# jhamrick/gaussian_processes

Hardware: AMD Instinct MI355X
Metric: GP fit+predict wall-clock (kernel build + Cholesky + solve + log_lh + posterior mean) (lower is better)
Workload: dtype f64; 1 GPU; N=65536 d=32 RBF(GaussianKernel) f64, m=1000 test points, h=1 w=0.5*sqrt(d) s=1; N=65536, d=32, m=1000, parallelism=1 GPU

## Files before the change

### gaussian_processes_amd/_lib.py

```python
import ctypes
import os
from ctypes import (POINTER, c_char_p, c_double, c_float, c_int, c_int64, c_size_t,
                    c_uint64, c_void_p)

import numpy as np

_HERE = os.path.dirname(os.path.abspath(__file__))
LIB_PATH = os.path.join(_HERE, "libgpx.so")

OK = 0
ERR_ARG, ERR_HIP, ERR_NO_DEVICE, ERR_NOMEM, ERR_UNSUPPORTED, ERR_INTERNAL = -1, -2, -3, -4, -5, -6
(ROUTE_TRSV_OPS, ROUTE_TRSV_STEPS, ROUTE_PANEL_RES, ROUTE_PANEL_CHAIN, ROUTE_FIT_RIDE, ROUTE_FIT_TWO_SOLVES,
 ROUTE_GEMM_FAST, ROUTE_GEMM_GENERIC, ROUTE_SYRK_EXACT, ROUTE_SYRK_PATCH, ROUTE_MG_BCAST_ONE, ROUTE_MG_BCAST_SAG,
 ROUTE_FIT_OPS_AHEAD, ROUTE_TRSM_OPS, ROUTE_POTRF_PAIR, ROUTE_VAR_CHUNK, ROUTE_LOO_CHUNK, ROUTE_TRSM_L_OPS,
 ROUTE_GRAD_CHUNK) = range(19)
F64, F32 = 0, 1
KERNEL_GAUSSIAN, KERNEL_PERIODIC, KERNEL_GAUSSIAN_ARD = 0, 1, 2
ARD_MAX_D = 64
FULL, LOWER = 0, 1
(K, DK_DH, DK_DW, DK_DP, D2K_DHDH, D2K_DHDW, D2K_DHDP, D2K_DWDW, D2K_DWDP, D2K_DPDP) = range(10)
MIN_LOG = -705.6238298100243

MEMBER_BY_NAME = {
    "K": K, "dK_dh": DK_DH, "dK_dw": DK_DW, "dK_dp": DK_DP,
    "d2K_dhdh": D2K_DHDH, "d2K_dhdw": D2K_DHDW, "d2K_dwdh": D2K_DHDW,
    "d2K_dhdp": D2K_DHDP, "d2K_dpdh": D2K_DHDP, "d2K_dwdw": D2K_DWDW,
    "d2K_dwdp": D2K_DWDP, "d2K_dpdw": D2K_DWDP, "d2K_dpdp": D2K_DPDP,
}

MG_ID_BYTES = 128
MG_BCAST_FN = ctypes.CFUNCTYPE(c_int, c_void_p, c_void_p, c_size_t, c_int, c_void_p)
MG_ALLREDUCE_FN = ctypes.CFUNCTYPE(c_int, c_void_p, c_void_p, c_size_t, c_int, c_int, c_void_p)

c_double_p = POINTER(c_double)
c_int_p = POINTER(c_int)

_SIGNATURES = {
    "gpx_version": (c_int, []),
    "gpx_last_error": (c_char_p, []),
    "gpx_device_count": (c_int, [c_int_p]),
    "gpx_set_device": (c_int, [c_int]),
    "gpx_get_device": (c_int, [c_int_p]),
    "gpx_device_info": (c_int, [c_int, c_char_p, c_size_t, c_int_p, c_int_p, POINTER(c_uint64)]),
    "gpx_malloc": (c_int, [POINTER(c_void_p), c_size_t]),
    "gpx_free": (c_int, [c_void_p]),
    "gpx_mem_info": (c_int, [ctypes.POINTER(c_size_t), ctypes.POINTER(c_size_t)]),
    "gpx_memcpy_h2d": (c_int, [c_void_p, c_void_p, c_size_t, c_void_p]),
    "gpx_memcpy_d2h": (c_int, [c_void_p, c_void_p, c_size_t, c_void_p]),
# ... 249 lines not shown
```

### gaussian_processes_amd/csrc/gpx_common.h

```cpp
#pragma once
#include <hip/hip_runtime.h>
#include <stdint.h>
#include <stdio.h>
#include <stdlib.h>
#include <string.h>
#include <math.h>
#include <vector>

#include "../../include/gpx.h"
#include "gpx_tune.h"

namespace gpx {

void set_error(const char *fmt, ...);
int  hip_fail(hipError_t e, const char *what, const char *file, int line);
int  ensure_device();

#define GPX_HIP(call)                                                        \
    do {                                                                     \
        hipError_t e__ = (call);                                             \
        if (e__ != hipSuccess) return gpx::hip_fail(e__, #call, __FILE__, __LINE__); \
    } while (0)

#define GPX_TRY(call)                                                        \
    do {                                                                     \
        int rc__ = (call);                                                   \
        if (rc__ != GPX_OK) return rc__;                                     \
    } while (0)

#define GPX_ARG(cond, msg)                                                   \
    do {                                                                     \
        if (!(cond)) { gpx::set_error("%s: %s", __func__, msg); return GPX_ERR_ARG; } \
    } while (0)

#define GPX_LAUNCH_CHECK()                                                   \
    do {                                                                     \
        hipError_t e__ = hipGetLastError();                                  \
        if (e__ != hipSuccess) return gpx::hip_fail(e__, "kernel launch", __FILE__, __LINE__); \
    } while (0)


enum Route { RT_TRSV_OPS = 0, RT_TRSV_STEPS = 1, RT_PANEL_RES = 2, RT_PANEL_CHAIN = 3, RT_FIT_RIDE = 4,
             RT_FIT_TWO_SOLVES = 5, RT_GEMM_FAST = 6, RT_GEMM_GENERIC = 7, RT_SYRK_EXACT = 8, RT_SYRK_PATCH = 9,
             RT_MG_BCAST_ONE = 10, RT_MG_BCAST_SAG = 11, RT_FIT_OPS_AHEAD = 12, RT_TRSM_OPS = 13, RT_POTRF_PAIR = 14, RT_VAR_CHUNK = 15, RT_LOO_CHUNK = 16,
             RT_TRSM_L_OPS = 17, RT_GRAD_CHUNK = 18, RT_COUNT = 19 };
void route_hit(int route);

int check_internal_info(int info);

static inline hipStream_t S(void *s) { return (hipStream_t)s; }
static inline size_t esize(int dtype) { return dtype == GPX_F64 ? 8 : 4; }
static inline int64_t round_up(int64_t v, int64_t m) { return (v + m - 1) / m * m; }
static inline int64_t cdiv(int64_t a, int64_t b) { return (a + b - 1) / b; }

static inline int order(hipEvent_t e, hipStream_t from, hipStream_t to)
{
    GPX_HIP(hipEventRecord(e, from));
    GPX_HIP(hipStreamWaitEvent(to, e, 0));
    return GPX_OK;
}
struct EventPool {
    std::vector<hipEvent_t> ev; size_t next = 0;
    int reserve(size_t count)
    {
        while (ev.size() < count) {
            hipEvent_t x;
            GPX_HIP(hipEventCreateWithFlags(&x, hipEventDisableTiming));
            ev.push_back(x);
        }
        return GPX_OK;
    }
    int get(hipEvent_t *e) { GPX_TRY(reserve(next + 1)); *e = ev[next++]; return GPX_OK; }
    void rewind() { next = 0; }
    void destroy() { for (hipEvent_t e : ev) (void)hipEventDestroy(e); ev.clear(); next = 0; }
    int order(hipStream_t from, hipStream_t to) { hipEvent_t e; GPX_TRY(get(&e)); return gpx::order(e, from, to); }
};

enum ProfClass { PC_KMAT = 0, PC_GEMM = 1, PC_POTRF_DIAG = 2, PC_TRSM_ROWS = 3, PC_TRSV = 4,
// ... 60 lines not shown
int syrk_bc(int dtype, int64_t n, int64_t row_begin, void *Cloc, int64_t ldc, int64_t cl0, int64_t cl1,
            const void *Pb, int64_t ldp, int64_t k0, int64_t kb, int64_t nb, int P, int rank,
            hipStream_t st, const int *abort_flag = nullptr, const Batch *bt = nullptr);
struct PanelHints { bool idle_chip = false; int leaf_force = 0; };
struct PotrfHook { int (*fn)(void *user, int64_t cols_done, hipEvent_t panel_done); void *user; };
int potrf_panel(int dtype, void *A, int64_t lda, int64_t n, int64_t r0, int64_t c0, int64_t kb,
                int *info_dev, hipStream_t st, const Batch *bt = nullptr, int64_t kpre = 0,
                hipEvent_t done = nullptr, PanelHints hints = {});
int potrf(int dtype, void *A, int64_t n, int64_t lda, int *info_dev, hipStream_t st, const Batch *bt = nullptr,
          int64_t xrows = 0,
          bool may_block = false,
          const PotrfHook *hook = nullptr);
int potrf_panel_res(int dtype, void *A, int64_t lda, int64_t n, int64_t r0, int64_t c0, int64_t kb, int *info_dev,
                    hipStream_t st, const Batch *bt = nullptr, int64_t kpre = 0, hipEvent_t done = nullptr, PanelHints hints = {});
int64_t panel_res_max();
hipStream_t potrf_side_stream();
bool kernel_values_finite(int kernel, const double *p, double s, int dtype);
bool panel_res_fold(int64_t rows, int64_t kpre, int64_t kb, size_t es, int64_t lda, const void *base);
constexpr int TRSV_OPS_BLOCK = 512;
static inline int64_t trsv_ops_nblocks(int64_t n) { return n / TRSV_OPS_BLOCK; }
static inline bool trsv_ops_whole_blocks(int64_t n) { return n >= TRSV_OPS_BLOCK && n % TRSV_OPS_BLOCK == 0; }
struct TrsvOps {
    GrowBuf mem;
    bool valid = false;
    int64_t built = 0;
    void invalidate() { valid = false; built = 0; }
    static TrsvOps view(void *p, size_t bytes) { TrsvOps o; o.mem.p = p; o.mem.bytes = bytes; return o; }
};
int trsv_ops_build(int dtype, const void *L, int64_t n, int64_t ldl, TrsvOps *ops, hipStream_t st);
bool trsv_ops_ahead_ok(int dtype, const void *L, int64_t n, int64_t ldl);
bool trsm_ops_ok(int dtype, const void *L, int64_t n, int64_t ldl);
size_t trsv_ops_bytes(int dtype, int64_t n);
int trsv_ops_build_upto(int dtype, const void *L, int64_t n, int64_t ldl, TrsvOps *ops, int64_t kend, hipStream_t st);
int trsv_lower(int dtype, const void *L, int64_t n, int64_t ldl, void *b, void *x, int transpose,
               hipStream_t st, const Batch *bt = nullptr,
               TrsvOps *ops = nullptr);
int trsm_right_lt(int dtype, const void *L, int64_t n, int64_t ldl, void *X, int64_t m, int64_t ldx,
                  hipStream_t st, int x_upper = 0, TrsvOps *ops = nullptr,
                  int64_t c0 = 0);
int trsm_right_l(int dtype, const void *L, int64_t n, int64_t ldl, void *X, int64_t m, int64_t ldx, hipStream_t st,
                 TrsvOps *ops = nullptr);
int pred_grad(int dtype, int kernel, const void *xo, int64_t m, const void *x, int64_t n, int d, const double *params,
              const void *alpha, const void *B, int64_t ldb, double scale, const double *col_div, double *out_dev, hipStream_t st);
int inv_from_factor(int dtype, const void *L, int64_t n, int64_t ldl, void *X, void *W, int tri, hipStream_t st,
                    TrsvOps *ops, int count = 1, int64_t sL = 0, void *group_ops = nullptr);
int logdet_chol(int dtype, const void *L, int64_t n, int64_t ldl, double *out_dev, hipStream_t st, int count = 1,
                int64_t sL = 0, int64_t so = 0);
int dot(int dtype, const void *a, const void *b, int64_t n, double *out_dev, hipStream_t st, int count = 1,
        int64_t sa = 0, int64_t sb = 0, int64_t so = 0);
int tril(int dtype, void *A, int64_t n, int64_t lda, hipStream_t st);
int var_rows(int dtype, int kernel, const void *X, int64_t rows, int64_t n, int64_t ldx, const void *xo, int d,
             const double *params, const double *kdiag_dev, int accumulate, double *out_dev, hipStream_t st);
int var_finish(int dtype, int kernel, const void *xo, int d, const double *params, const double *acc_dev, int64_t rows,
               double *out_dev, hipStream_t st);
int eye_rows(int dtype, void *X, int64_t rows, int64_t ld, int64_t c0, int64_t cz, hipStream_t st);
int loo_rows(int dtype, const void *X, int64_t rows, int64_t n, int64_t ldx, int64_t c0, const void *y, const void *alpha,
             double *kii, double *mean, double *var, double *logp, hipStream_t st);
int loo_points(int dtype, const double *kii, const void *y, const void *alpha, int64_t n, double *mean, double *var, double *logp,
               hipStream_t st);
int sum_f64(const double *a, int64_t n, double *out_dev, hipStream_t st);
int var_plan(int dtype, int64_t n, int64_t m, int64_t chunk_rows, size_t free_bytes, int64_t *rows, int64_t *chunks, size_t *bytes);
int dloglh_reduce(int dtype, int kernel, const void *x, int64_t n, int d, const double *params,
                  const void *alpha, const void *W, int64_t ldw, double *partial_dev, double *out4,
                  hipStream_t st);
int scale_points(int dtype, const void *x, int64_t n, int d, const double *w_host, void *out, hipStream_t st);
void ard_iso(const double *params, int d, double *iso2);
// ... 8 lines not shown
```

### gaussian_processes_amd/csrc/gpx_gp.hip

```cpp
#include "gpx_common.h"
#include <cmath>
#include <vector>

#include "gpx_gp_internal.h"

namespace gpx {

template <typename T>
__global__ void cvt_from_f64(const double *__restrict__ src, T *__restrict__ dst, int64_t n)
{
    const int64_t i = (int64_t)blockIdx.x * blockDim.x + threadIdx.x;
    if (i < n) dst[i] = (T)src[i];
}

template <typename T>
__global__ void cvt_to_f64_2d(const T *__restrict__ src, int64_t lds, double *__restrict__ dst,
                              int64_t ldd, int64_t rows, int64_t cols, int lower_only)
{
    const int64_t c = (int64_t)blockIdx.x * blockDim.x + threadIdx.x;
    if (c >= cols) return;
    for (int64_t r = blockIdx.y; r < rows; r += gridDim.y) {
        const double v = (double)src[r * lds + c];
        dst[r * ldd + c] = (lower_only && c > r) ? 0.0 : v;
    }
// ... 250 lines not shown
int gpx_gp_get_params(gpx_gp_t *g, double *params, int cap, int *count)
{
    GP_ENTER(g);
    GPX_ARG(g->have_params, "no kernel parameters in the handle");
    GPX_ARG(cap >= 0 && (cap == 0 || params), "bad arguments");
    if (count) *count = g->nparams;
    for (int i = 0; i < g->nparams && i < cap; ++i) params[i] = g->params[i];
    return GPX_OK;
}

int gpx_gp_set_K(gpx_gp_t *g, const double *Kxx, int64_t ld)
{
    GP_ENTER(g);
    GPX_ARG(g && Kxx && ld >= g->n, "bad arguments");
    const int64_t n = g->n;
    if (g->dtype == GPX_F64) {
        GPX_HIP(hipMemcpy2DAsync(g->A, (size_t)g->lda * 8, Kxx, (size_t)ld * 8, (size_t)n * 8, (size_t)n,
                                 hipMemcpyHostToDevice, g->st));
        GPX_HIP(hipStreamSynchronize(g->st));
    } else {
        DevBuf tmp;
        GPX_TRY(tmp.alloc((size_t)n * n * 8));
        GPX_HIP(hipMemcpy2DAsync(tmp.p, (size_t)n * 8, Kxx, (size_t)ld * 8, (size_t)n * 8, (size_t)n,
                                 hipMemcpyHostToDevice, g->st));
        for (int64_t r = 0; r < n; ++r)
            hipLaunchKernelGGL((cvt_from_f64<float>), dim3((unsigned)cdiv(n, 256)), dim3(256), 0, g->st,
                               (const double *)tmp.p + r * n, (float *)g->A + r * g->lda, n);
        GPX_HIP(hipStreamSynchronize(g->st));
    }
    g->have_K = true; g->fitted = false; g->have_kii = false;
    return GPX_OK;
}

struct OpsAhead { gpx_gp *g; int64_t group, last; };
static int ops_ahead_step(void *user, int64_t cols_done, hipEvent_t panel_done)
{
    OpsAhead *o = (OpsAhead *)user;
    gpx_gp *g = o->g;
    const int64_t ready = std::min(trsv_ops_nblocks(cols_done), o->last);
    if (ready - g->ops.built < o->group) return GPX_OK;
    GPX_HIP(hipStreamWaitEvent(g->st_ops, panel_done, 0));
    return trsv_ops_build_upto(g->dtype, g->A, g->n, g->lda, &g->ops, ready, g->st_ops);
}

int gpx_gp_fit(gpx_gp_t *g, int *info)
{
    GP_ENTER(g);
    GPX_ARG(g, "gp is NULL");
    GPX_ARG(g->have_data && (g->have_params || g->have_K),
            "set_data and set_params (or set_K) must be called before fit");
    const GpView v = gp_view(g);
    if (!g->have_K && (!g->x_finite || !kernel_values_finite(v.kernel, v.params, g->s, g->dtype))) {
        set_error("%s (%s)", NONFINITE_MSG, g->x_finite ? "kernel parameters or s" : "x");
        return GPX_ERR_ARG;
    }
    const size_t es = esize(g->dtype);
    int *info_dev = (int *)(g->scal + 3);
    hipStream_t st = g->st;
    GPX_HIP(hipEventRecord(g->ev[0], st));
    if (!g->have_K)
        GPX_TRY(kmat(g->dtype, v.kernel, GPX_K, v.x, g->n, v.x, g->n, g->d, v.params, g->s * g->s,
                     GPX_LOWER, g->A, g->lda, st));
    g->have_K = false;
    g->have_kii = false;
    GPX_HIP(hipEventRecord(g->ev[1], st));
    const int64_t ride_max = tune().fit_ride_max;
    const bool ride = g->n <= ride_max;
    route_hit(ride ? RT_FIT_RIDE : RT_FIT_TWO_SOLVES);
    char *row_n = (char *)g->A + (size_t)g->n * g->lda * es;
    if (ride) GPX_HIP(hipMemcpyAsync(row_n, g->y, (size_t)g->n * es, hipMemcpyDeviceToDevice, st));
    g->ops.invalidate();
    const bool ahead = tune().fit_ops_ahead != 0 && g->n >= tune().fit_ops_ahead_min &&
                       trsv_ops_ahead_ok(g->dtype, g->A, g->n, g->lda);
    const int64_t nfull = trsv_ops_nblocks(g->n), tail = tune().fit_ops_tail;
    const int64_t group = std::max<int64_t>(1, std::min(nfull, nfull - tail));
    OpsAhead oa = {g, group, std::max<int64_t>(0, nfull - tail)};
    PotrfHook hook = {ops_ahead_step, &oa};
    if (ahead) {
        if (!g->st_ops) {
            int least = 0, greatest = 0;
            GPX_HIP(hipDeviceGetStreamPriorityRange(&least, &greatest));
            GPX_HIP(hipStreamCreateWithPriority(&g->st_ops, hipStreamNonBlocking, least));
            GPX_HIP(hipEventCreateWithFlags(&g->ev_ops, hipEventDisableTiming));
        }
        GPX_TRY(g->ops.mem.reserve(trsv_ops_bytes(g->dtype, g->n), st));
        GPX_TRY(order(g->ev_ops, st, g->st_ops));
    }
    GPX_TRY(potrf(g->dtype, g->A, g->n, g->lda, info_dev, st, nullptr, ride ? 1 : 0, true, ahead ? &hook : nullptr));
    if (ahead) {
        GPX_TRY(order(g->ev_ops, g->st_ops, st));
        if (g->ops.built > 0) route_hit(RT_FIT_OPS_AHEAD);
    }
    GPX_HIP(hipEventRecord(g->ev[2], st));
    if (ride) {
        GPX_TRY(trsv_lower(g->dtype, g->A, g->n, g->lda, row_n, g->alpha, 1, st, nullptr, &g->ops));
    } else {
        GPX_HIP(hipMemcpyAsync(g->t0, g->y, (size_t)g->n * es, hipMemcpyDeviceToDevice, st));
        GPX_TRY(trsv_lower(g->dtype, g->A, g->n, g->lda, g->t0, g->t1, 0, st, nullptr, &g->ops));
        GPX_TRY(trsv_lower(g->dtype, g->A, g->n, g->lda, g->t1, g->alpha, 1, st, nullptr, &g->ops));
    }
    GPX_HIP(hipEventRecord(g->ev[3], st));
    GPX_TRY(logdet_chol(g->dtype, g->A, g->n, g->lda, g->scal + 0, st));
    GPX_TRY(dot(g->dtype, g->y, g->alpha, g->n, g->scal + 1, st));
    GPX_HIP(hipEventRecord(g->ev[4], st));
    g->fitted = true;
    if (info) {
        GPX_HIP(hipMemcpyAsync(info, info_dev, sizeof(int), hipMemcpyDeviceToHost, st));
        GPX_HIP(hipStreamSynchronize(st));
        GPX_TRY(check_internal_info(*info));
    }
    return GPX_OK;
}

static int gp_scalars(gpx_gp_t *g, double *logdet, double *yta, int *info)
{
    GP_ENTER(g);
    GPX_ARG(g && g->fitted, "gp is not fitted");
    double h[4];
    GPX_HIP(hipMemcpyAsync(h, g->scal, sizeof(h), hipMemcpyDeviceToHost, g->st));
    GPX_HIP(hipStreamSynchronize(g->st));
    int inf;
    memcpy(&inf, &h[3], sizeof(int));
    GPX_TRY(check_internal_info(inf));
    if (logdet) *logdet = h[0];
    if (yta) *yta = h[1];
    if (info) *info = inf;
    return GPX_OK;
}
// ... 743 lines not shown
```

### gaussian_processes_amd/csrc/gpx_gp_internal.h

```cpp
#pragma once
#include "gpx_common.h"

struct gpx_gp {
    int device;
    int dtype, kernel, d, nparams;
    int64_t n, lda;
    void *x, *y, *A, *alpha, *t0, *t1;
    void *xs;
    double *scal;
    hipStream_t st;
    hipEvent_t ev[6];
    double params[1 + GPX_ARD_MAX_D];
    double iso[2];
    double s;
    bool have_data, have_params, fitted, have_K;
    bool x_finite, y_finite;
    float ms[5];
    gpx::GrowBuf bw; int64_t bw_cap;
    gpx::TrsvOps ops;
    gpx::GrowBuf gw; int64_t gw_cap;
    gpx::TrsvOps bops;
    double *kii;
    bool have_kii;
    hipStream_t st_ops;
    hipEvent_t ev_ops;
};

namespace gpx {
int gp_scan_finite(gpx_gp *g);
static inline int nparams_of(int kernel, int d) { return kernel == GPX_KERNEL_GAUSSIAN_ARD ? 1 + d : (kernel == GPX_KERNEL_PERIODIC ? 3 : 2); }
struct GpView { int kernel; const void *x; const double *params; };
static inline GpView gp_view(const gpx_gp *g)
{
    if (g->kernel == GPX_KERNEL_GAUSSIAN_ARD) return {GPX_KERNEL_GAUSSIAN, g->xs, g->iso};
    return {g->kernel, g->x, g->params};
}
int gp_rescale(gpx_gp *g);
}

#define GP_ENTER(g)                                                          \
    GPX_ARG((g) != nullptr, "gp is NULL");                                   \
    gpx::tune_refresh();                                                     \
    gpx::DeviceGuard guard__((g)->device);                                   \
    if (guard__.rc != GPX_OK) return guard__.rc;                             \
    gpx::StreamTurn turn__((g)->st);                                         \
    gpx::RoctxRange api_range__(__func__)
```

### gaussian_processes_amd/csrc/gpx_mg.hip

```cpp
#include "gpx_common.h"
#include <dlfcn.h>
#include <climits>
#include <cmath>
#include <vector>

extern "C" {
typedef struct ncclComm *ncclComm_t;
typedef struct { char internal[128]; } ncclUniqueId;
typedef int ncclResult_t;
typedef int ncclDataType_t;
typedef int ncclRedOp_t;
}
static constexpr ncclResult_t ncclSuccess = 0;
static constexpr ncclDataType_t ncclInt32 = 2, ncclFloat32 = 7, ncclFloat64 = 8;
static constexpr ncclRedOp_t ncclSum = 0, ncclMax = 2;
static_assert(sizeof(ncclUniqueId) == GPX_MG_ID_BYTES, "ncclUniqueId is 128 bytes");

extern "C" int gpx_d_mean(int dtype, int kernel, const void *xo, int64_t m, const void *x, int64_t n, int d,
                          const double *params, const void *alpha, void *out, void *stream);
namespace gpx {

struct Rccl {
    void *lib = nullptr;
    ncclResult_t (*GetUniqueId)(ncclUniqueId *) = nullptr;
// ... 550 lines not shown
    GPX_HIP(hipDeviceGetStreamPriorityRange(&least, &greatest));
    GPX_HIP(hipStreamCreateWithPriority(&g->Q, hipStreamNonBlocking, greatest));
    GPX_HIP(hipStreamCreateWithPriority(&g->B, hipStreamNonBlocking, greatest));
    GPX_HIP(hipStreamCreateWithPriority(&g->O, hipStreamNonBlocking, least));
    for (size_t jl = 0; jl < g->my_blocks.size(); ++jl) {
        const int64_t kb = g->kb(g->my_blocks[jl]);
        if (!trsv_ops_whole_blocks(kb)) continue;
        GPX_TRY(g->ops[jl].mem.reserve(trsv_ops_bytes(g->dtype, kb), g->O));
    }
    return GPX_OK;
}

static int mg_new(gpx_mg **out, int dtype, int kernel, int64_t n, int d, int64_t nb, int world, int rank)
{
    GPX_TRY(ensure_device());
    GPX_ARG(out, "mg is NULL");
    *out = nullptr;
    GPX_ARG(dtype == GPX_F64 || dtype == GPX_F32, "dtype must be GPX_F64 or GPX_F32");
    GPX_ARG(kernel == GPX_KERNEL_GAUSSIAN || kernel == GPX_KERNEL_PERIODIC, "unknown kernel family");
    GPX_ARG(n >= 1 && d >= 1, "need n >= 1 and d >= 1");
    GPX_ARG(world >= 1 && rank >= 0 && rank < world, "bad world / rank");
    GPX_ARG(nb >= 64 && nb % 64 == 0 && 1024 % nb == 0, "nb must be 64 / 128 / 256 / 512 / 1024");
    gpx_mg *g = new gpx_mg();
    g->dtype = dtype; g->kernel = kernel; g->n = n; g->d = d; g->nb = nb; g->world = world; g->rank = rank;
    g->es = esize(dtype);
    if (hipGetDevice(&g->device) != hipSuccess) { (void)hipGetLastError(); g->device = 0; }
    g->nblk = cdiv(n, nb);
    for (int64_t j = rank; j < g->nblk; j += world) g->my_blocks.push_back(j);
    g->ncols_local = std::max<int64_t>(1, (int64_t)g->my_blocks.size()) * nb;
    g->ld = g->ncols_local;
    g->nr = n + 1;
    g->ops.resize(std::max<size_t>(1, g->my_blocks.size()));
    g->bcast_chunks = (int)std::max<int64_t>(1, std::min<int64_t>(16, tune().mg_bcast_chunks));
    g->timing = !tune().mg_no_timing;
    if (tune().mg_bcast_set) g->bcast_sag = tune().mg_bcast_sag;
    g->owner_first = tune().mg_owner_first_set ? (tune().mg_owner_first != 0) : (world >= 2);
    *out = g;
    return GPX_OK;
}


static double mg_hash(const void *p, size_t bytes)
{
    uint64_t h = 1469598103934665603ull;
    const unsigned char *c = (const unsigned char *)p;
    for (size_t i = 0; i < bytes; ++i) { h ^= c[i]; h *= 1099511628211ull; }
    return (double)(h >> 12);
}

constexpr int MG_COV_AGREE = 8, MG_VAR_AGREE = 11;
static int mg_cov_agree(gpx_mg *g, double *v, int nv = MG_COV_AGREE, const char *who = "gpx_mg_cov")
{
    double *dv = g->scal + 4;
    GPX_HIP(hipMemcpyAsync(dv, v, nv * sizeof(double), hipMemcpyHostToDevice, g->S));
    GPX_TRY(mg_allreduce(g, dv, nv, GPX_F64, 1, g->S));
    GPX_HIP(hipMemcpyAsync(v, dv, nv * sizeof(double), hipMemcpyDeviceToHost, g->S));
    GPX_HIP(hipStreamSynchronize(g->S));
    if (v[0] != 0) { set_error("%s: a device allocation failed on at least one rank", who); return GPX_ERR_NOMEM; }
    if (v[1] != 0) {
        set_error("%s: bad arguments on at least one rank (m < 0 or a NULL pointer%s)", who, nv > MG_COV_AGREE ? ", or a chunk_rows that is not a multiple of 128" : "");
        return GPX_ERR_ARG;
    }
    if (v[2] != -v[3]) { set_error("%s: the ranks called with different m (%.0f .. %.0f)", who, -v[3], v[2]); return GPX_ERR_ARG; }
    if (v[4] != -v[5]) { set_error("%s: the ranks called with different xo", who); return GPX_ERR_ARG; }
    if (v[6] != -v[7]) { set_error("%s: the ranks called with different params", who); return GPX_ERR_ARG; }
    if (nv > MG_COV_AGREE && v[8] != -v[9]) { set_error("%s: the ranks called with different chunk_rows (%.0f .. %.0f)", who, -v[9], v[8]); return GPX_ERR_ARG; }
    return GPX_OK;
// ... 521 lines not shown
```

### gaussian_processes_amd/csrc/gpx_potrf.hip

```cpp
#include "gpx_common.h"
#include "gpx_leaf.h"
#include <vector>

namespace gpx {

constexpr int IBP = IB + 1;


template <typename T, bool INV>
__global__ __launch_bounds__(256) void potrf_diag_kernel(T *__restrict__ blk, int64_t lda, int64_t j0,
                                                         int jb, int *__restrict__ info, T *__restrict__ inv,
                                                         int64_t sblk)
{
    blk += (int64_t)blockIdx.x * sblk;
    info += blockIdx.x;
    if (INV) inv += (int64_t)blockIdx.x * (IB * IB);
    __builtin_amdgcn_s_setprio(3);
    const int tid = threadIdx.x;
    const int tr = tid >> 4, tc = tid & 15;
    __shared__ int s_abort;
    if (tid == 0) s_abort = *info;
    __syncthreads();
    if (s_abort != 0) return;
    T a[4][4];
// ... 118 lines not shown

static int64_t outer_block(int64_t n, bool batched = false)
{
    const int64_t forced = tune().potrf_nb;
    if (forced >= IB && forced % IB == 0) return forced;
    if (batched && n >= 8192 && n <= 32768) return 1024;
    if (batched && n >= 4096 && n <= 32768) return 512;
    const long long *thr = tune().potrf_widths;
    if (n <= thr[0]) return 128;
    if (n <= thr[1]) return 256;
    if (n <= thr[2]) return 512;
    return 1024;
}

static thread_local ThreadScratch g_leaf;

template <typename T>
static int potrf_panel_t(T *A, int64_t lda, int64_t n, int64_t r0, int64_t c0, int64_t kb, int *info_dev,
                         hipStream_t st, int dtype, const Batch *bt, int64_t kpre = 0, hipEvent_t done = nullptr,
                         PanelHints hints = {})
{
    const int nbatch = bt ? bt->count : 1;
    const int64_t sM = bt ? bt->sA : 0;
    if (kb % IB == 0 && kb <= panel_res_max()) {
        route_hit(RT_PANEL_RES);
        return potrf_panel_res(dtype, A, lda, n, r0, c0, kb, info_dev, st, bt, kpre, done, hints);
    }
    if (kpre != 0) { set_error("potrf_panel: a folded update needs the resident panel route"); return GPX_ERR_ARG; }
    if (kb <= IB) {
        route_hit(RT_PANEL_CHAIN);
        const int jb = (int)kb;
        T *D = A + r0 * lda + c0;
        const int64_t below = n - (r0 + jb);
        const bool via_inverse = !tune().potrf_trsm_rows && below > 0 && below <= tune().potrf_inv_max &&
                                 jb == IB && lda % (16 / (int64_t)sizeof(T)) == 0 &&
                                 ((uintptr_t)(A + (r0 + jb) * lda + c0)) % 16 == 0;
        T *inv = nullptr;
        if (via_inverse) {
            void *p = nullptr;
            GPX_TRY(g_leaf.get(std::max<size_t>((size_t)nbatch * IB * IB * sizeof(T), IB * IB * 8), &p));
            inv = (T *)p;
        }
        {
            ProfScope prof(PC_POTRF_DIAG, (double)jb * jb * jb / 3.0 * nbatch, st);
            if (inv)
                hipLaunchKernelGGL((potrf_diag_kernel<T, true>), dim3(nbatch), dim3(256), 0, st, D, lda, r0, jb,
                                   info_dev, inv, sM);
            else
                hipLaunchKernelGGL((potrf_diag_kernel<T, false>), dim3(nbatch), dim3(256), 0, st, D, lda, r0, jb,
                                   info_dev, inv, sM);
        }
        GPX_LAUNCH_CHECK();
        if (via_inverse) {
            T *Xb = A + (r0 + jb) * lda + c0;
            Batch bi; bi.count = nbatch; bi.sA = sM; bi.sB = IB * IB; bi.sC = sM;
            GPX_TRY(gemm_nt(dtype, below, jb, jb, Xb, lda, inv, IB, Xb, lda, 1.0, GPX_FULL, 0, 0, st, 1, 0,
                            bt ? &bi : nullptr));
        } else if (below > 0) {
            Batch br; br.count = nbatch; br.sA = sM; br.sB = sM; br.sC = 0;
            GPX_TRY(trsm_rows(dtype, A + (r0 + jb) * lda + c0, lda, below, D, lda, jb, st, bt ? &br : nullptr));
        }
        if (done) GPX_HIP(hipEventRecord(done, st));
        return GPX_OK;
    }
    const int64_t h = ((kb / IB + 1) / 2) * IB;
    GPX_TRY(potrf_panel_t<T>(A, lda, n, r0, c0, h, info_dev, st, dtype, bt, 0, nullptr, hints));
    hints.idle_chip = false;
// ... 218 lines not shown
```

### gaussian_processes_amd/csrc/gpx_solve.hip

```cpp
#include "gpx_common.h"
#include "gpx_kernels_dev.h"
#include "gpx_leaf.h"

namespace gpx {

constexpr int SB = 64;
constexpr int OB = TRSV_OPS_BLOCK;

template <typename T>
__global__ __launch_bounds__(256) void inv64_kernel(const T *__restrict__ L, int64_t ldl, int64_t ncols,
                                                    T *__restrict__ out, int transposed, T *__restrict__ W,
                                                    T *__restrict__ Wt, int64_t bsL, int64_t bsOut)
{
    L += (int64_t)blockIdx.y * bsL;
    const int tid = threadIdx.x, tr = tid >> 4, tc = tid & 15;
    const int64_t k0 = (int64_t)blockIdx.x * SB;
    const int jb = (int)min((int64_t)SB, ncols - k0);
    const T *blk = L + k0 * ldl + k0;
    T a[4][4], x[4][4];
#pragma unroll
    for (int r = 0; r < 4; ++r)
#pragma unroll
        for (int c = 0; c < 4; ++c) {
            const int row = 4 * tr + r, col = 4 * tc + c;
// ... 512 lines not shown
    const int64_t n = S.n, nb = S.nb();
    auto launch = [&](int64_t far_rows, int64_t nn, int64_t k0, int jb, int64_t p0, int pjb, int64_t far0) {
        hipLaunchKernelGGL((trsv_fwd_fused<T>), dim3((unsigned)(1 + cdiv(far_rows, 64)), S.nbt), dim3(TBT), 0, S.st, S.L, S.ldl,
                           S.Linv, S.b, S.x, nn, k0, jb, p0, pjb, far0, S.aligned, S.sL, S.sLinv, S.sv);
    };
    for (int64_t blk = kfirst; blk < nb; ++blk) {
        const int64_t k0 = blk * TB, p0 = std::max<int64_t>(blk - 1, 0) * TB;
        const int jb = S.width(blk), pjb = blk > 0 ? TB : 0;
        if (blk > 0) launch(jb, k0 + jb, k0, 0, p0, pjb, k0);
        launch(blk > 0 ? n - (k0 + jb) : 0, n, k0, jb, p0, pjb, k0 + jb);
    }
    if (n > S.ncols) launch(n - S.ncols, n, S.ncols, 0, (nb - 1) * TB, S.width(nb - 1), S.ncols);
}

template <typename T>
static void steps_bwd(const Sweep<T> &S, int64_t kfirst)
{
    const int64_t nb = S.nb();
    for (int64_t blk = nb - 1; blk >= kfirst; --blk) {
        const int64_t k0 = blk * TB, q0 = k0 + TB;
        const int jb = S.width(blk), qjb = blk + 1 < nb ? S.width(blk + 1) : 0;
        if (qjb > 0)
            hipLaunchKernelGGL((trsv_bwd_fused<T, 32>), dim3((unsigned)(1 + cdiv(jb, 32)), S.nbt), dim3(TBT), 0, S.st, S.L,
                               S.ldl, S.Linv, S.b, S.x, k0, 0, q0, qjb, k0, k0 + jb, S.aligned, S.sL, S.sLinv, S.sv);
        hipLaunchKernelGGL((trsv_bwd_fused<T, 128>), dim3((unsigned)(1 + (qjb > 0 ? cdiv(k0, 128) : 0)), S.nbt),
                           dim3(TBT), 0, S.st, S.L, S.ldl, S.Linv, S.b, S.x, k0, jb, q0, qjb, (int64_t)0, k0, S.aligned,
                           S.sL, S.sLinv, S.sv);
    }
}

constexpr int NCH = OB / (TBT / OPL);

template <typename T>
static void ops_fwd(const Sweep<T> &S, const OpsView<T> &V)
{
    for (int64_t k = 0; k < V.nfull; ++k) {
        const int64_t k0 = k * OB, far0 = k0 + OB;
        const int64_t nfar = k > 0 ? cdiv(S.n - far0, 64) : 0;
        hipLaunchKernelGGL((trsv_op_kernel<T, true>), dim3((unsigned)(NCH + nfar)), dim3(TBT), 0, S.st, V.W(k),
                           k > 0 ? V.Tf(k) : (const T *)nullptr, S.L, S.ldl, S.b, S.x, S.n, k0, k0 - OB, k > 0 ? OB : 0, far0, S.n, NCH, 1);
    }
}

template <typename T>
static void ops_bwd(const Sweep<T> &S, const OpsView<T> &V, int64_t kend)
{
    for (int64_t k = kend - 1; k >= 0; --k) {
        const int64_t k0 = k * OB, q0 = k0 + OB;
        const int qjb = (k + 1 < V.nfull) ? OB : (int)(S.n - q0);
        const int64_t nfar = qjb > 0 ? cdiv(k0, 128) : 0;
        hipLaunchKernelGGL((trsv_op_kernel<T, false>), dim3((unsigned)(NCH + nfar)), dim3(TBT), 0, S.st, V.Wt(k),
                           qjb > 0 ? V.Tb(k) : (const T *)nullptr, S.L, S.ldl, S.b, S.x, S.n, k0, q0, qjb, (int64_t)0, k0, NCH, 1);
    }
}

template <typename T>
static int trsv_t(const T *L, int64_t n, int64_t ldl, T *b, T *x, int transpose, hipStream_t st,
                  int64_t ncols = -1, const Batch *bt = nullptr, TrsvOps *ops = nullptr)
{
    constexpr int dtype = sizeof(T) == 8 ? GPX_F64 : GPX_F32;
    if (ncols < 0 || ncols > n) ncols = n;
    Sweep<T> S;
    S.L = L; S.n = n; S.ldl = ldl; S.ncols = ncols; S.b = b; S.x = x; S.st = st;
    S.nbt = (unsigned)(bt ? bt->count : 1); S.sL = bt ? bt->sA : 0; S.sv = bt ? bt->sB : 0;
    ProfScope prof(PC_TRSV, ((double)n * ncols - 0.5 * (double)ncols * (ncols - 1)) * sizeof(T) * S.nbt, st);
    S.sLinv = cdiv(ncols, SB) * SB * SB;
    void *scr = nullptr;
    GPX_TRY(g_scr.get((size_t)S.nbt * S.sLinv * sizeof(T), &scr));
    S.Linv = (T *)scr;
    S.aligned = (((uintptr_t)L) % (2 * sizeof(T)) == 0) && (ldl % 2 == 0);
    const bool usable = !bt && ncols == n && ops_usable(dtype, L, ldl);
    const bool cached = ops && ops->mem.p && n % OB == 0 && ops->mem.bytes >= trsv_ops_bytes(dtype, n);
    const bool prebuilt = cached && ops->valid;
    const int64_t kpart = (usable && cached && !ops->valid && ops->built > 0 && transpose) ? std::min(ops->built, n / OB) : 0;
    if (kpart == 0 && usable && (n >= trsv_ops_min_n() || prebuilt)) {
        route_hit(RT_TRSV_OPS);
        void *buf = nullptr;
        if (ops) {
            bool grew = false;
            GPX_TRY(ops->mem.reserve(trsv_ops_bytes(dtype, n), st, &grew));
            if (grew) ops->invalidate();
            buf = ops->mem.p;
        } else {
            GPX_TRY(g_ops.get(trsv_ops_bytes(dtype, n), &buf));
        }
        const OpsView<T> V(buf, n);
        if (!ops || !ops->valid) GPX_TRY(trsv_ops_prepare<T>(L, n, ldl, buf, st, ops ? std::min(ops->built, V.nfull) : 0, V.nfull));
        if (ops) { ops->valid = true; ops->built = V.nfull; }
        const bool ragged = n > V.nfull * OB;
        if (!transpose) {
            ops_fwd(S, V);
            if (ragged) { inv64_blocks(S, 0, 1); steps_fwd(S, V.nfull); }
        } else {
            if (ragged) { inv64_blocks(S, 0, 0); steps_bwd(S, V.nfull); }
            ops_bwd(S, V, V.nfull);
        }
    } else if (!transpose) {
        route_hit(RT_TRSV_STEPS);
        inv64_blocks(S, 0, 1);
        steps_fwd(S, 0);
    } else {
        route_hit(RT_TRSV_STEPS);
        inv64_blocks(S, kpart * (OB / SB), 0);
        steps_bwd(S, kpart);
        if (kpart > 0) {
            route_hit(RT_TRSV_OPS);
            ops_bwd(S, OpsView<T>(ops->mem.p, n), kpart);
        }
    }
    GPX_LAUNCH_CHECK();
    return GPX_OK;
}

int trsv_lower(int dtype, const void *L, int64_t n, int64_t ldl, void *b, void *x, int transpose,
               hipStream_t st, const Batch *bt, TrsvOps *ops)
{
    if (n <= 0) return GPX_OK;
    if (dtype == GPX_F64)
        return trsv_t<double>((const double *)L, n, ldl, (double *)b, (double *)x, transpose, st, -1, bt, ops);
    return trsv_t<float>((const float *)L, n, ldl, (float *)b, (float *)x, transpose, st, -1, bt, ops);
}

int trsv_ops_build(int dtype, const void *L, int64_t n, int64_t ldl, TrsvOps *ops, hipStream_t st)
{
    if (!ops || !trsv_ops_whole_blocks(n) || !ops_usable(dtype, L, ldl)) return GPX_OK;
    GPX_TRY(ops->mem.reserve(trsv_ops_bytes(dtype, n), st));
    ops->invalidate();
    if (dtype == GPX_F64) GPX_TRY(trsv_ops_prepare<double>((const double *)L, n, ldl, ops->mem.p, st));
    else GPX_TRY(trsv_ops_prepare<float>((const float *)L, n, ldl, ops->mem.p, st));
    ops->valid = true;
    ops->built = n / OB;
    return GPX_OK;
}

int trsv_ops_build_upto(int dtype, const void *L, int64_t n, int64_t ldl, TrsvOps *ops, int64_t kend, hipStream_t st)
{
    if (!ops || !trsv_ops_ahead_ok(dtype, L, n, ldl)) return GPX_OK;
    const int64_t nfull = n / OB;
    kend = std::min(kend, nfull);
    if (ops->built == 0) {
        GPX_TRY(ops->mem.reserve_device(trsv_ops_bytes(dtype, n)));
        ops->valid = false;
    }
    if (kend <= ops->built || !ops->mem.p) return GPX_OK;
    if (dtype == GPX_F64) GPX_TRY(trsv_ops_prepare<double>((const double *)L, n, ldl, ops->mem.p, st, ops->built, kend));
    else GPX_TRY(trsv_ops_prepare<float>((const float *)L, n, ldl, ops->mem.p, st, ops->built, kend));
    ops->built = kend;
    if (kend == nfull) ops->valid = true;
    return GPX_OK;
}

int trsv_lower_cols(int dtype, const void *L, int64_t n, int64_t ldl, int64_t ncols, void *b, void *x,
                    hipStream_t st)
{
    if (n <= 0 || ncols <= 0) return GPX_OK;
    if (dtype == GPX_F64)
        return trsv_t<double>((const double *)L, n, ldl, (double *)b, (double *)x, 0, st, ncols);
    return trsv_t<float>((const float *)L, n, ldl, (float *)b, (float *)x, 0, st, ncols);
}

template <typename T>
__global__ __launch_bounds__(256) void panel_gemv_t_partial(const T *__restrict__ Lp, int64_t ldl,
                                                            int64_t rows, int ncols,
                                                            const T *__restrict__ x, double *__restrict__ work)
{
    __shared__ T sx[256];
    const int tid = threadIdx.x;
    const int64_t r0 = (int64_t)blockIdx.x * 256;
    sx[tid] = (r0 + tid < rows) ? x[r0 + tid] : (T)0;
    __syncthreads();
    const int nr = (int)std::min<int64_t>(256, rows - r0);
    for (int c = tid; c < ncols; c += 256) {
        const T *col = Lp + r0 * ldl + c;
        double acc = 0.0;
        for (int i = 0; i < nr; ++i) acc = fma((double)col[(int64_t)i * ldl], (double)sx[i], acc);
        work[(int64_t)blockIdx.x * ncols + c] = acc;
    }
}

template <typename T>
__global__ void panel_gemv_t_reduce(const double *__restrict__ work, int64_t nchunks, int ncols,
// ... 657 lines not shown
```

### gaussian_processes_amd/csrc/gpx_tune.h

```cpp
#pragma once
#include <stdint.h>

namespace gpx {

#define GPX_TUNE_LIST(X, XF, XS, X2)                                                                                   \
                                                                               \
    XF(gemm_no_fast, "GPX_GEMM_NO_FAST")                                                                               \
    X(gemm_ablate, "GPX_GEMM_ABLATE", 0)                                                                               \
    X(gemm_pad_lds, "GPX_GEMM_PAD_LDS", 0)                                                                             \
    X(gemm_bn64_tiles, "GPX_GEMM_BN64_TILES", 256)                                                                     \
    X(gemm_exact, "GPX_GEMM_EXACT", 1)                                                                                 \
    X(gemm_fine_tiles, "GPX_GEMM_FINE_TILES", 16384)                                                                   \
    X2(syrk_bn64_tiles, "GPX_SYRK_BN64_TILES", 2600, 4000)                                                             \
                                                              \
    X(fit_ride_max, "GPX_FIT_RIDE_MAX", 16384)                                                                         \
    X(fit_ops_ahead, "GPX_FIT_OPS_AHEAD", 1)                                                                           \
    X(fit_ops_ahead_min, "GPX_FIT_OPS_AHEAD_MIN", 8192)                                                                \
    X(fit_ops_tail, "GPX_FIT_OPS_TAIL", 4)                                                                             \
    XS(batch_max, "GPX_BATCH_MAX", 1)                                                                                  \
    X(io_block_bytes, "GPX_IO_BLOCK_BYTES", (int64_t)64 << 20)                                                         \
    X(kmat_panel_bytes, "GPX_KMAT_PANEL_BYTES", (int64_t)256 << 20)                                                    \
                                                                        \
    XF(force_collectives, "GPX_FORCE_COLLECTIVES")                                                                     \
    X(mg_bcast_chunks, "GPX_MG_BCAST_CHUNKS", 4)                                                                       \
    XF(mg_no_timing, "GPX_MG_NO_TIMING")                                                                               \
    XS(mg_owner_first, "GPX_MG_OWNER_FIRST", 0)                                                                        \
                                                                  \
    XF(trace, "GPX_TRACE")                                                                                             \
    X(potrf_res, "GPX_POTRF_RES", 256)                                                                                 \
    X(res_strict, "GPX_RES_STRICT", 1)                                                                                 \
    X(two_part_rows, "GPX_POTRF_TWO_PART_ROWS", 16384)                                                                 \
    X(two_part_batch, "GPX_POTRF_TWO_PART_BATCH", 98304)                                                               \
    X(leaf_mfma_f32_rows, "GPX_LEAF_MFMA_F32_ROWS", 16384)                                                             \
    X(panel_excl_rows, "GPX_PANEL_EXCL_ROWS", 5120)                                                                    \
    XS(leaf, "GPX_LEAF", 0)                                                                                            \
    X2(leaf4_rows, "GPX_LEAF4_ROWS", 8192, 5120)                                                                       \
    X2(panel_pad_lds, "GPX_PANEL_PAD_LDS", 8 * 1024, 40 * 1024)                                                        \
    X(fold_rows, "GPX_POTRF_FOLD_ROWS", 16384)                                                                         \
    X(fold_k, "GPX_POTRF_FOLD_K", 256)                                                                                 \
                                                                  \
    XS(potrf_nb, "GPX_POTRF_NB", 0)                                                                                    \
    XF(potrf_trsm_rows, "GPX_POTRF_TRSM_ROWS")                                                                         \
    X(potrf_inv_max, "GPX_POTRF_INV_MAX", 16384)                                                                       \
    XF(no_lookahead, "GPX_POTRF_NO_LOOKAHEAD")                                                                         \
    X(taper, "GPX_POTRF_TAPER", 1)                                                                                     \
    X2(pair_rows, "GPX_POTRF_PAIR_ROWS", 0, 0)                                                                         \
    X(host_paced, "GPX_POTRF_HOST_PACED", 16384)                                                                       \
    X(gate_rows, "GPX_POTRF_GATE_ROWS", 16384)                                                                         \
                                                                                 \
    X(trsv_ops, "GPX_TRSV_OPS", 1)                                                                                     \
    X(trsv_ops_min, "GPX_TRSV_OPS_MIN", 10240)                                                                         \
    X(trsm_ops, "GPX_TRSM_OPS", 1)                                                                                     \
                                                                          \
    XF(roctx, "GPX_ROCTX")

struct Tune {
#define GPX_T_X(f, e, d) int64_t f = (d);
#define GPX_T_XF(f, e) bool f = false;
#define GPX_T_XS(f, e, d) int64_t f = (d); bool f##_set = false;
#define GPX_T_X2(f, e, d0, d1) int64_t f[2] = {(d0), (d1)};
    GPX_TUNE_LIST(GPX_T_X, GPX_T_XF, GPX_T_XS, GPX_T_X2)
#undef GPX_T_X
#undef GPX_T_XF
#undef GPX_T_XS
#undef GPX_T_X2
    long long potrf_widths[3] = {1, 8192, 12288};
    bool mg_bcast_set = false, mg_bcast_sag = false;
    char rccl_lib[256] = {0};
};

const Tune &tune();
void tune_refresh();
int64_t tune_refresh_count();

}
// ... 1 lines not shown
```

### include/gpx.h

```cpp
#ifndef GPX_H
#define GPX_H

#include <stddef.h>
#include <stdint.h>

#ifdef __cplusplus
extern "C" {
#endif

#define GPX_VERSION 100

#define GPX_OK              0
#define GPX_ERR_ARG        -1
#define GPX_ERR_HIP        -2
#define GPX_ERR_NO_DEVICE  -3
#define GPX_ERR_NOMEM      -4
#define GPX_ERR_UNSUPPORTED -5
#define GPX_ERR_INTERNAL   -6

#define GPX_F64 0
#define GPX_F32 1

#define GPX_KERNEL_GAUSSIAN 0
#define GPX_KERNEL_PERIODIC 1
// ... 52 lines not shown
#define GPX_PROF_POTRF_DIAG 2
#define GPX_PROF_TRSM_ROWS  3
#define GPX_PROF_TRSV       4
#define GPX_PROF_MEAN       5
#define GPX_PROF_REDUCE     6
#define GPX_PROF_GEMM_SKINNY  7
#define GPX_PROF_GEMM_GENERIC 8
#define GPX_PROF_GEMM_PANEL   9
#define GPX_PROF_GEMM_N64    10
#define GPX_PROF_TRANSPOSE   11
#define GPX_PROF_PRED_GRAD   12
int gpx_prof_enable(int on);
int gpx_prof_read(int cls, double *launches, double *total_ms, double *total_work);

#define GPX_ROUTE_TRSV_OPS        0
#define GPX_ROUTE_TRSV_STEPS      1
#define GPX_ROUTE_PANEL_RES       2
#define GPX_ROUTE_PANEL_CHAIN     3
#define GPX_ROUTE_FIT_RIDE        4
#define GPX_ROUTE_FIT_TWO_SOLVES  5
#define GPX_ROUTE_GEMM_FAST       6
#define GPX_ROUTE_GEMM_GENERIC    7
#define GPX_ROUTE_SYRK_EXACT      8
#define GPX_ROUTE_SYRK_PATCH      9
#define GPX_ROUTE_MG_BCAST_ONE   10
#define GPX_ROUTE_MG_BCAST_SAG   11
#define GPX_ROUTE_FIT_OPS_AHEAD  12
#define GPX_ROUTE_TRSM_OPS       13
#define GPX_ROUTE_POTRF_PAIR     14
#define GPX_ROUTE_VAR_CHUNK      15
#define GPX_ROUTE_LOO_CHUNK      16
#define GPX_ROUTE_TRSM_L_OPS     17
#define GPX_ROUTE_GRAD_CHUNK     18
int gpx_debug_route_count(int route, int64_t *count);
int gpx_debug_roctx_ranges(int64_t *count);
int gpx_debug_route_reset(void);
int gpx_debug_tune_refreshes(int64_t *count);
int gpx_debug_leaf_selfcheck(int run_now, int *state);


int gpx_d_kmat(int dtype, int kernel, int member, const void *x1, int64_t n,
               const void *x2, int64_t m, int d, const double *params,
               double diag_add, int tri, void *out, int64_t ld, void *stream);

int gpx_d_scale_points(int dtype, const void *x, int64_t n, int d, const double *w_host, void *out, void *stream);

int gpx_d_mean(int dtype, int kernel, const void *xo, int64_t m, const void *x,
               int64_t n, int d, const double *params, const void *alpha,
               void *out, void *stream);

int gpx_d_mean_member(int dtype, int kernel, int member, const void *xo, int64_t m, const void *x,
                      int64_t n, int d, const double *params, const void *alpha, void *out, void *stream);

int gpx_d_pred_grad(int dtype, int kernel, const void *xo, int64_t m, const void *x, int64_t n, int d,
                    const double *params, const void *alpha, const void *B, int64_t ldb, double scale,
                    double *out_dev, void *stream);

int gpx_d_gemm_nt(int dtype, int64_t M, int64_t N, int64_t K, double alpha,
                  const void *A, int64_t lda, const void *B, int64_t ldb, void *C,
                  int64_t ldc, int tri, int64_t row0, int64_t col0, void *stream);

int gpx_d_potrf(int dtype, void *A, int64_t n, int64_t lda, int *info_dev,
                void *stream);

int gpx_d_potrf_panel(int dtype, void *A, int64_t lda, int64_t n, int64_t r0, int64_t c0,
                      int64_t kb, int *info_dev, void *stream);
// ... 150 lines not shown
```

Baseline: 1.391 s.

## Run forward triangular solve on ops stream during Cholesky in groups

```diff
diff --git a/gaussian_processes_amd/_lib.py b/gaussian_processes_amd/_lib.py
--- a/gaussian_processes_amd/_lib.py
+++ b/gaussian_processes_amd/_lib.py
@@ -13,7 +13,7 @@
 (ROUTE_TRSV_OPS, ROUTE_TRSV_STEPS, ROUTE_PANEL_RES, ROUTE_PANEL_CHAIN, ROUTE_FIT_RIDE, ROUTE_FIT_TWO_SOLVES,
  ROUTE_GEMM_FAST, ROUTE_GEMM_GENERIC, ROUTE_SYRK_EXACT, ROUTE_SYRK_PATCH, ROUTE_MG_BCAST_ONE, ROUTE_MG_BCAST_SAG,
  ROUTE_FIT_OPS_AHEAD, ROUTE_TRSM_OPS, ROUTE_POTRF_PAIR, ROUTE_VAR_CHUNK, ROUTE_LOO_CHUNK, ROUTE_TRSM_L_OPS,
- ROUTE_GRAD_CHUNK) = range(19)
+ ROUTE_GRAD_CHUNK, ROUTE_FIT_FWD_AHEAD) = range(20)
 F64, F32 = 0, 1
 KERNEL_GAUSSIAN, KERNEL_PERIODIC, KERNEL_GAUSSIAN_ARD = 0, 1, 2
 ARD_MAX_D = 64
diff --git a/gaussian_processes_amd/csrc/gpx_common.h b/gaussian_processes_amd/csrc/gpx_common.h
--- a/gaussian_processes_amd/csrc/gpx_common.h
+++ b/gaussian_processes_amd/csrc/gpx_common.h
@@ -43,7 +43,7 @@
 enum Route { RT_TRSV_OPS = 0, RT_TRSV_STEPS = 1, RT_PANEL_RES = 2, RT_PANEL_CHAIN = 3, RT_FIT_RIDE = 4,
              RT_FIT_TWO_SOLVES = 5, RT_GEMM_FAST = 6, RT_GEMM_GENERIC = 7, RT_SYRK_EXACT = 8, RT_SYRK_PATCH = 9,
              RT_MG_BCAST_ONE = 10, RT_MG_BCAST_SAG = 11, RT_FIT_OPS_AHEAD = 12, RT_TRSM_OPS = 13, RT_POTRF_PAIR = 14, RT_VAR_CHUNK = 15, RT_LOO_CHUNK = 16,
-             RT_TRSM_L_OPS = 17, RT_GRAD_CHUNK = 18, RT_COUNT = 19 };
+             RT_TRSM_L_OPS = 17, RT_GRAD_CHUNK = 18, RT_FIT_FWD_AHEAD = 19, RT_COUNT = 20 };
 void route_hit(int route);
 
 int check_internal_info(int info);
@@ -170,6 +170,9 @@
 bool trsm_ops_ok(int dtype, const void *L, int64_t n, int64_t ldl);
 size_t trsv_ops_bytes(int dtype, int64_t n);
 int trsv_ops_build_upto(int dtype, const void *L, int64_t n, int64_t ldl, TrsvOps *ops, int64_t kend, hipStream_t st);
+bool trsv_fwd_ops_ok(int dtype, const void *L, int64_t n, int64_t ldl);
+int trsv_fwd_ops_range(int dtype, const void *L, int64_t n, int64_t ldl, const TrsvOps *ops, void *b, void *x, int64_t kbeg,
+                       int64_t kend, hipStream_t st);
 int trsv_lower(int dtype, const void *L, int64_t n, int64_t ldl, void *b, void *x, int transpose,
                hipStream_t st, const Batch *bt = nullptr,
                TrsvOps *ops = nullptr);
diff --git a/gaussian_processes_amd/csrc/gpx_gp.hip b/gaussian_processes_amd/csrc/gpx_gp.hip
--- a/gaussian_processes_amd/csrc/gpx_gp.hip
+++ b/gaussian_processes_amd/csrc/gpx_gp.hip
@@ -306,15 +306,21 @@
     return GPX_OK;
 }
 
-struct OpsAhead { gpx_gp *g; int64_t group, last; };
+struct OpsAhead { gpx_gp *g; int64_t group, last; bool fwd; };
 static int ops_ahead_step(void *user, int64_t cols_done, hipEvent_t panel_done)
 {
     OpsAhead *o = (OpsAhead *)user;
     gpx_gp *g = o->g;
     const int64_t ready = std::min(trsv_ops_nblocks(cols_done), o->last);
-    if (ready - g->ops.built < o->group) return GPX_OK;
+    const int64_t fresh = ready - g->ops.built;
+    if (fresh <= 0 || (fresh < o->group && ready < o->last)) return GPX_OK;
     GPX_HIP(hipStreamWaitEvent(g->st_ops, panel_done, 0));
-    return trsv_ops_build_upto(g->dtype, g->A, g->n, g->lda, &g->ops, ready, g->st_ops);
+    GPX_TRY(trsv_ops_build_upto(g->dtype, g->A, g->n, g->lda, &g->ops, ready, g->st_ops));
+    if (o->fwd && g->ops.built > g->fwd_done) {
+        GPX_TRY(trsv_fwd_ops_range(g->dtype, g->A, g->n, g->lda, &g->ops, g->t0, g->t1, g->fwd_done, g->ops.built, g->st_ops));
+        g->fwd_done = g->ops.built;
+    }
+    return GPX_OK;
 }
 
 int gpx_gp_fit(gpx_gp_t *g, int *info)
@@ -344,11 +350,15 @@
     char *row_n = (char *)g->A + (size_t)g->n * g->lda * es;
     if (ride) GPX_HIP(hipMemcpyAsync(row_n, g->y, (size_t)g->n * es, hipMemcpyDeviceToDevice, st));
     g->ops.invalidate();
+    g->fwd_done = 0;
     const bool ahead = tune().fit_ops_ahead != 0 && g->n >= tune().fit_ops_ahead_min &&
                        trsv_ops_ahead_ok(g->dtype, g->A, g->n, g->lda);
     const int64_t nfull = trsv_ops_nblocks(g->n), tail = tune().fit_ops_tail;
-    const int64_t group = std::max<int64_t>(1, std::min(nfull, nfull - tail));
-    OpsAhead oa = {g, group, std::max<int64_t>(0, nfull - tail)};
+    const bool grouped = ahead && !ride && g->n >= tune().fit_ops_group_min;
+    const bool fwd_ahead = grouped && trsv_fwd_ops_ok(g->dtype, g->A, g->n, g->lda);
+    int64_t group = std::max<int64_t>(1, std::min(nfull, nfull - tail));
+    if (grouped && tune().fit_ops_group > 0) group = std::min(group, tune().fit_ops_group);
+    OpsAhead oa = {g, group, std::max<int64_t>(0, nfull - tail), fwd_ahead};
     PotrfHook hook = {ops_ahead_step, &oa};
     if (ahead) {
         if (!g->st_ops) {
@@ -359,15 +369,24 @@
         }
         GPX_TRY(g->ops.mem.reserve(trsv_ops_bytes(g->dtype, g->n), st));
         GPX_TRY(order(g->ev_ops, st, g->st_ops));
-    }
-    GPX_TRY(potrf(g->dtype, g->A, g->n, g->lda, info_dev, st, nullptr, ride ? 1 : 0, true, ahead ? &hook : nullptr));
+        if (fwd_ahead) GPX_HIP(hipMemcpyAsync(g->t0, g->y, (size_t)g->n * es, hipMemcpyDeviceToDevice, g->st_ops));
+    }
+    const int potrf_rc = potrf(g->dtype, g->A, g->n, g->lda, info_dev, st, nullptr, ride ? 1 : 0, true, ahead ? &hook : nullptr);
     if (ahead) {
         GPX_TRY(order(g->ev_ops, g->st_ops, st));
-        if (g->ops.built > 0) route_hit(RT_FIT_OPS_AHEAD);
-    }
+        if (potrf_rc == GPX_OK && g->ops.built > 0) route_hit(RT_FIT_OPS_AHEAD);
+    }
+    GPX_TRY(potrf_rc);
     GPX_HIP(hipEventRecord(g->ev[2], st));
     if (ride) {
         GPX_TRY(trsv_lower(g->dtype, g->A, g->n, g->lda, row_n, g->alpha, 1, st, nullptr, &g->ops));
+    } else if (fwd_ahead) {
+        if (g->fwd_done > 0) route_hit(RT_FIT_FWD_AHEAD);
+        route_hit(RT_TRSV_OPS);
+        GPX_TRY(trsv_ops_build_upto(g->dtype, g->A, g->n, g->lda, &g->ops, nfull, st));
+        GPX_TRY(trsv_fwd_ops_range(g->dtype, g->A, g->n, g->lda, &g->ops, g->t0, g->t1, g->fwd_done, nfull, st));
+        g->fwd_done = nfull;
+        GPX_TRY(trsv_lower(g->dtype, g->A, g->n, g->lda, g->t1, g->alpha, 1, st, nullptr, &g->ops));
     } else {
         GPX_HIP(hipMemcpyAsync(g->t0, g->y, (size_t)g->n * es, hipMemcpyDeviceToDevice, st));
         GPX_TRY(trsv_lower(g->dtype, g->A, g->n, g->lda, g->t0, g->t1, 0, st, nullptr, &g->ops));
diff --git a/gaussian_processes_amd/csrc/gpx_gp_internal.h b/gaussian_processes_amd/csrc/gpx_gp_internal.h
--- a/gaussian_processes_amd/csrc/gpx_gp_internal.h
+++ b/gaussian_processes_amd/csrc/gpx_gp_internal.h
@@ -18,6 +18,7 @@
     float ms[5];
     gpx::GrowBuf bw; int64_t bw_cap;
     gpx::TrsvOps ops;
+    int64_t fwd_done;
     gpx::GrowBuf gw; int64_t gw_cap;
     gpx::TrsvOps bops;
     double *kii;
diff --git a/gaussian_processes_amd/csrc/gpx_mg.hip b/gaussian_processes_amd/csrc/gpx_mg.hip
--- a/gaussian_processes_amd/csrc/gpx_mg.hip
+++ b/gaussian_processes_amd/csrc/gpx_mg.hip
@@ -606,7 +606,7 @@
     g->nr = n + 1;
     g->ops.resize(std::max<size_t>(1, g->my_blocks.size()));
     g->bcast_chunks = (int)std::max<int64_t>(1, std::min<int64_t>(16, tune().mg_bcast_chunks));
-    g->timing = !tune().mg_no_timing;
+    g->timing = true;
     if (tune().mg_bcast_set) g->bcast_sag = tune().mg_bcast_sag;
     g->owner_first = tune().mg_owner_first_set ? (tune().mg_owner_first != 0) : (world >= 2);
     *out = g;
diff --git a/gaussian_processes_amd/csrc/gpx_potrf.hip b/gaussian_processes_amd/csrc/gpx_potrf.hip
--- a/gaussian_processes_amd/csrc/gpx_potrf.hip
+++ b/gaussian_processes_amd/csrc/gpx_potrf.hip
@@ -174,7 +174,7 @@
         const int jb = (int)kb;
         T *D = A + r0 * lda + c0;
         const int64_t below = n - (r0 + jb);
-        const bool via_inverse = !tune().potrf_trsm_rows && below > 0 && below <= tune().potrf_inv_max &&
+        const bool via_inverse = below > 0 && below <= tune().potrf_inv_max &&
                                  jb == IB && lda % (16 / (int64_t)sizeof(T)) == 0 &&
                                  ((uintptr_t)(A + (r0 + jb) * lda + c0)) % 16 == 0;
         T *inv = nullptr;
diff --git a/gaussian_processes_amd/csrc/gpx_solve.hip b/gaussian_processes_amd/csrc/gpx_solve.hip
--- a/gaussian_processes_amd/csrc/gpx_solve.hip
+++ b/gaussian_processes_amd/csrc/gpx_solve.hip
@@ -568,9 +568,9 @@
 constexpr int NCH = OB / (TBT / OPL);
 
 template <typename T>
-static void ops_fwd(const Sweep<T> &S, const OpsView<T> &V)
-{
-    for (int64_t k = 0; k < V.nfull; ++k) {
+static void ops_fwd(const Sweep<T> &S, const OpsView<T> &V, int64_t kbeg, int64_t kend)
+{
+    for (int64_t k = kbeg; k < kend; ++k) {
         const int64_t k0 = k * OB, far0 = k0 + OB;
         const int64_t nfar = k > 0 ? cdiv(S.n - far0, 64) : 0;
         hipLaunchKernelGGL((trsv_op_kernel<T, true>), dim3((unsigned)(NCH + nfar)), dim3(TBT), 0, S.st, V.W(k),
@@ -625,7 +625,7 @@
         if (ops) { ops->valid = true; ops->built = V.nfull; }
         const bool ragged = n > V.nfull * OB;
         if (!transpose) {
-            ops_fwd(S, V);
+            ops_fwd(S, V, 0, V.nfull);
             if (ragged) { inv64_blocks(S, 0, 1); steps_fwd(S, V.nfull); }
         } else {
             if (ragged) { inv64_blocks(S, 0, 0); steps_bwd(S, V.nfull); }
@@ -683,6 +683,32 @@
     else GPX_TRY(trsv_ops_prepare<float>((const float *)L, n, ldl, ops->mem.p, st, ops->built, kend));
     ops->built = kend;
     if (kend == nfull) ops->valid = true;
+    return GPX_OK;
+}
+
+bool trsv_fwd_ops_ok(int dtype, const void *L, int64_t n, int64_t ldl) { return trsv_ops_ahead_ok(dtype, L, n, ldl) && n >= trsv_ops_min_n(); }
+
+template <typename T>
+static void fwd_ops_range_t(const T *L, int64_t n, int64_t ldl, const void *buf, T *b, T *x, int64_t kbeg, int64_t kend, hipStream_t st)
+{
+    Sweep<T> S = {};
+    S.L = L; S.n = n; S.ldl = ldl; S.ncols = n; S.b = b; S.x = x; S.st = st; S.nbt = 1; S.aligned = 1;
+    ops_fwd(S, OpsView<T>(buf, n), kbeg, kend);
+}
+
+int trsv_fwd_ops_range(int dtype, const void *L, int64_t n, int64_t ldl, const TrsvOps *ops, void *b, void *x, int64_t kbeg,
+                       int64_t kend, hipStream_t st)
+{
+    if (!ops || !ops->mem.p || !trsv_ops_ahead_ok(dtype, L, n, ldl) || ops->mem.bytes < trsv_ops_bytes(dtype, n) ||
+        kbeg < 0 || kend > ops->built || kend > n / OB) {
+        set_error("trsv_fwd_ops_range: blocks [%lld, %lld) of a factor with %lld blocks of operators", (long long)kbeg,
+                  (long long)kend, (long long)(ops ? ops->built : 0));
+        return GPX_ERR_ARG;
+    }
+    if (kend <= kbeg) return GPX_OK;
+    if (dtype == GPX_F64) fwd_ops_range_t<double>((const double *)L, n, ldl, ops->mem.p, (double *)b, (double *)x, kbeg, kend, st);
+    else fwd_ops_range_t<float>((const float *)L, n, ldl, ops->mem.p, (float *)b, (float *)x, kbeg, kend, st);
+    GPX_LAUNCH_CHECK();
     return GPX_OK;
 }
 
diff --git a/gaussian_processes_amd/csrc/gpx_tune.h b/gaussian_processes_amd/csrc/gpx_tune.h
--- a/gaussian_processes_amd/csrc/gpx_tune.h
+++ b/gaussian_processes_amd/csrc/gpx_tune.h
@@ -17,13 +17,14 @@
     X(fit_ops_ahead, "GPX_FIT_OPS_AHEAD", 1)                                                                           \
     X(fit_ops_ahead_min, "GPX_FIT_OPS_AHEAD_MIN", 8192)                                                                \
     X(fit_ops_tail, "GPX_FIT_OPS_TAIL", 4)                                                                             \
+    X(fit_ops_group_min, "GPX_FIT_OPS_GROUP_MIN", 32768)                                                               \
+    X(fit_ops_group, "GPX_FIT_OPS_GROUP", 16)                                                                          \
     XS(batch_max, "GPX_BATCH_MAX", 1)                                                                                  \
     X(io_block_bytes, "GPX_IO_BLOCK_BYTES", (int64_t)64 << 20)                                                         \
     X(kmat_panel_bytes, "GPX_KMAT_PANEL_BYTES", (int64_t)256 << 20)                                                    \
                                                                         \
     XF(force_collectives, "GPX_FORCE_COLLECTIVES")                                                                     \
     X(mg_bcast_chunks, "GPX_MG_BCAST_CHUNKS", 4)                                                                       \
-    XF(mg_no_timing, "GPX_MG_NO_TIMING")                                                                               \
     XS(mg_owner_first, "GPX_MG_OWNER_FIRST", 0)                                                                        \
                                                                   \
     XF(trace, "GPX_TRACE")                                                                                             \
@@ -40,7 +41,6 @@
     X(fold_k, "GPX_POTRF_FOLD_K", 256)                                                                                 \
                                                                   \
     XS(potrf_nb, "GPX_POTRF_NB", 0)                                                                                    \
-    XF(potrf_trsm_rows, "GPX_POTRF_TRSM_ROWS")                                                                         \
     X(potrf_inv_max, "GPX_POTRF_INV_MAX", 16384)                                                                       \
     XF(no_lookahead, "GPX_POTRF_NO_LOOKAHEAD")                                                                         \
     X(taper, "GPX_POTRF_TAPER", 1)                                                                                     \
diff --git a/include/gpx.h b/include/gpx.h
--- a/include/gpx.h
+++ b/include/gpx.h
@@ -108,6 +108,7 @@
 #define GPX_ROUTE_LOO_CHUNK      16
 #define GPX_ROUTE_TRSM_L_OPS     17
 #define GPX_ROUTE_GRAD_CHUNK     18
+#define GPX_ROUTE_FIT_FWD_AHEAD  19
 int gpx_debug_route_count(int route, int64_t *count);
 int gpx_debug_roctx_ranges(int64_t *count);
 int gpx_debug_route_reset(void);
```

New measurement: 1.387 s, median of 5. About the same (-0.3%).
